# matschiner/navier-stokes-solver

Measured on AMD Instinct MI355X. Metric: Krylov iters/sec, 3D SIMPLE Stokes solve (BPCG), higher is better.
Workload: dtype f64

## Files before the change

### navier-stokes-solver_amd/csrc/bpcg2.hip

```cpp
#include "dist.h"


namespace nss {

enum { S_WD = 0, S_AS = 1, S_WDN = 2, S_ALPHA = 3, S_BETA = 4, S_ERR0 = 5, S_TOL = 6, S_REL = 7, S_WD_ODD = 8,
       S_AS_LOCAL = 9, S_WDN_LOCAL = 10 };
__device__ __forceinline__ int wd_slot(int it) { return (it & 1) ? S_WD_ODD : S_WD; }
enum { C_DONE = 0, C_IT_FINAL = 1, C_LAST_IT = 2, C_BREAKDOWN = 3, C_PENDING = 4, C_COMPUTED = 5, C_CLOSED = 6 };

struct EpiK1 {
  const int32_t* __restrict__ ctrl;
  const double* __restrict__ scal;
  double* __restrict__ u0;
  double* __restrict__ q;
  double* __restrict__ z0;
  const double* __restrict__ t2;
  double* __restrict__ s0;
  const double* __restrict__ w0;
  double* __restrict__ t0;
  double* __restrict__ t1;
  const double* __restrict__ dinv;
  double k;
  int it;
  __device__ bool skip() const { return ctrl[C_DONE] != 0; }
// ... 296 lines not shown
      u.x = fma(alpha, sv.x, u.x);
      u.y = fma(alpha, sv.y, u.y);
      double2 dn, wn;
      dn.x = fma(-alpha, t3v.x, d.x);
      dn.y = fma(-alpha, t3v.y, d.y);
      wn.x = fma(-alpha, mv.x * t3v.x, w.x);
      wn.y = fma(-alpha, mv.y * t3v.y, w.y);
      *reinterpret_cast<double2*>(a.u1 + i0) = u;
      *reinterpret_cast<double2*>(a.d1 + i0) = dn;
      *reinterpret_cast<double2*>(a.w1 + i0) = wn;
      acc = fma(wn.x, dn.x, acc);
      acc = fma(wn.y, dn.y, acc);
    } else {
      for (int i = i0; i < i0 + 2 && i < a.n_p; ++i) {
        const double sv = a.s1[i], t3v = a.t3[i];
        a.u1[i] = fma(alpha, sv, a.u1[i]);
        const double dn = fma(-alpha, t3v, a.d1[i]);
        const double wn = fma(-alpha, a.minv[i] * t3v, a.w1[i]);
        a.d1[i] = dn;
        a.w1[i] = wn;
        acc = fma(wn, dn, acc);
      }
    }
  } else {
    const int first = wg - a.gu - a.gp, stride = (int(gridDim.x) - a.gu - a.gp) * kBlock;
    for (int i = first * kBlock + int(threadIdx.x); i < a.ghost_n; i += stride)
      a.ghost_w0[i] = fma(-alpha, a.t1[a.ghost_map ? a.ghost_map[i] : a.n_u + i], a.ghost_w0[i]);
    for (int i = first * kBlock + int(threadIdx.x); i < a.ghost_p_n; i += stride)
      a.ghost_w1[i] = fma(-alpha, a.ghost_minv[i] * a.ghost_t3[i], a.ghost_w1[i]);
    return;
  }
  store_block_partial(acc, wg, a.partials, lds);
}

__global__ __launch_bounds__(kBlock) void bpcg2_k5_kernel(int32_t* __restrict__ ctrl, double* __restrict__ scal,
                                                           double* __restrict__ hist, int32_t it, int32_t n_p,
                                                           double* __restrict__ s1, const double* __restrict__ w1,
                                                           int32_t ghost_n, double* __restrict__ ghost_s0,
                                                           const double* __restrict__ ghost_w0, int32_t ghost_p_n,
                                                           double* __restrict__ ghost_s1,
                                                           const double* __restrict__ ghost_w1) {
  if (ctrl[C_DONE] != 0) return;
  const double wd = scal[wd_slot(it)], wdn = scal[S_WDN];
  const double beta = wdn / wd;
  if (blockIdx.x == 0 && threadIdx.x == 0) {
    scal[S_BETA] = beta;
    scal[wd_slot(it + 1)] = wdn;
    const double err = sqrt(fabs(wd));
    hist[it] = err;
    ctrl[C_LAST_IT] = it;
    ctrl[C_CLOSED] = it + 1;
    const double bound = scal[S_TOL] * (scal[S_REL] != 0.0 ? scal[S_ERR0] : 1.0);
    if (err < bound) {
      ctrl[C_IT_FINAL] = it;
      ctrl[C_DONE] = 1;
    }
  }
  const int stride = gridDim.x * kBlock;
  for (int i = blockIdx.x * kBlock + threadIdx.x; i < n_p; i += stride) s1[i] = fma(beta, s1[i], w1[i]);
  for (int i = blockIdx.x * kBlock + threadIdx.x; i < ghost_n; i += stride) ghost_s0[i] = fma(beta, ghost_s0[i], ghost_w0[i]);
  for (int i = blockIdx.x * kBlock + threadIdx.x; i < ghost_p_n; i += stride) ghost_s1[i] = fma(beta, ghost_s1[i], ghost_w1[i]);
}

__global__ __launch_bounds__(kBlock) void bpcg2_flush_kernel(const int32_t* __restrict__ ctrl,
                                                              const double* __restrict__ scal, int32_t n_u,
                                                              const double* __restrict__ s0, double* __restrict__ u0) {
  if (ctrl[C_PENDING] == 0) return;
  const double alpha = scal[S_ALPHA];
  const int stride = gridDim.x * kBlock;
  for (int i = blockIdx.x * kBlock + threadIdx.x; i < n_u; i += stride) u0[i] = fma(alpha, s0[i], u0[i]);
}

__global__ void bpcg2_flush_done_kernel(int32_t* __restrict__ ctrl) { ctrl[C_PENDING] = 0; }

struct CloseArgs {
  int32_t* ctrl;
  double* scal;
  double* hist;
  const double* partials_c;
  int32_t nc;
  int32_t fold;
};

template <bool FOLD>
__device__ __forceinline__ bool close_iteration(const CloseArgs& a, int it, double* lds, double* beta_out) {
  const int prev = it - 1;
  double wdn;
  if constexpr (FOLD) wdn = fixed_sum_1024(a.partials_c, a.nc, a.partials_c, 0, lds);
  else wdn = a.scal[S_WDN];
  const double wd = a.scal[wd_slot(prev)];
  const double beta = wdn / wd;
  const double err = sqrt(fabs(wd));
  const double bound = a.scal[S_TOL] * (a.scal[S_REL] != 0.0 ? a.scal[S_ERR0] : 1.0);
  const bool stop = err < bound;
  if (blockIdx.x == 0 && threadIdx.x == 0) {
    a.scal[S_BETA] = beta;
    a.scal[wd_slot(it)] = wdn;
    if (FOLD) a.scal[S_WDN] = wdn;
    a.hist[prev] = err;
    a.ctrl[C_LAST_IT] = prev;
    a.ctrl[C_CLOSED] = it;
    if (stop) {
      a.ctrl[C_IT_FINAL] = prev;
      a.ctrl[C_DONE] = 1;
    }
  }
  *beta_out = beta;
  return !stop;
}

__global__ __launch_bounds__(kBlock) void bpcg2_close_kernel(CloseArgs a) {
  __shared__ double lds[kRedDoubles];
  if (a.ctrl[C_DONE] != 0) return;
  const int computed = a.ctrl[C_COMPUTED];
  if (a.ctrl[C_CLOSED] >= computed) return;
  double beta;
  if (a.fold) close_iteration<true>(a, computed, lds, &beta);
  else close_iteration<false>(a, computed, lds, &beta);
}

template <bool FOLD, bool NT = false>
struct EpiK1c {
  CloseArgs cl;
  double* __restrict__ u0;
  double* __restrict__ q;
  double* __restrict__ z0;
  const double* __restrict__ t2;
  double* __restrict__ s0;
  const double* __restrict__ w0;
  double* __restrict__ t0;
  double* __restrict__ t1;
  const double* __restrict__ dinv;
  double k;
  int it;
  const double* __restrict__ s1;
  const double* __restrict__ w1;
  int32_t ghost_n = 0;
  double* __restrict__ ghost_s0 = nullptr;
  const double* __restrict__ ghost_w0 = nullptr;
  const int32_t* __restrict__ jb_first = nullptr;
  const int32_t* __restrict__ jb_order = nullptr;
  const int32_t* __restrict__ jb_run = nullptr;
  const double* __restrict__ jb_packed = nullptr;
  int32_t jb_count = 0, jb_bs = 0;
  double alpha = 0.0, beta = 0.0;
  bool pending = false;
  __device__ bool skip() const { return cl.ctrl[C_DONE] != 0; }
  __device__ bool prologue(double* lds) {
    if (it == 0) return true;
    alpha = cl.scal[S_ALPHA];
    pending = cl.ctrl[C_PENDING] == it;
    return close_iteration<FOLD>(cl, it, lds, &beta);
  }
  struct X {
    const double* __restrict__ s1;
    const double* __restrict__ w1;
    double beta;
    bool first;
    static constexpr bool kStageable = false;
    static constexpr bool kStageablePair = true;
    __device__ const double* ptr() const { return s1; }
    __device__ const double* ptr2() const { return w1; }
    __device__ double pair(double s, double w) const { return first ? s : fma(beta, s, w); }
    __device__ double operator()(int c) const { return first ? s1[c] : fma(beta, s1[c], w1[c]); }
  };
  __device__ X xop(const double*) const { return X{s1, w1, beta, it == 0}; }
#ifndef NSS_K1C_PREFETCH
#define NSS_K1C_PREFETCH 0
#endif

#if NSS_K1C_PREFETCH
  struct Pre { double q = 0.0, z0 = 0.0, t2 = 0.0, s0 = 0.0, w0 = 0.0, u0 = 0.0; };
  __device__ Pre fetch(int r) const {
    if (it == 0) return Pre{q[r], 0.0, 0.0, 0.0, 0.0, 0.0};
    return Pre{q[r], z0[r], t2[r], s0[r], w0[r], u0[r]};
  }
  __device__ void row(int r, double bts, const Pre& p) const {
#else
  struct PreLate { double q, z0, t2, s0, w0, u0; };
  __device__ void row(int r, double bts) const {
    const PreLate p{ld1s<NT>(q + r), it ? ld1s<NT>(z0 + r) : 0.0, it ? ld1s<NT>(t2 + r) : 0.0, it ? s0[r] : 0.0,
                    it ? ld1s<NT>(w0 + r) : 0.0, (it && pending) ? ld1s<NT>(u0 + r) : 0.0};
#endif
    double qv = p.q;
    if (it != 0) {
      const double zo = p.z0, t2v = p.t2, so = p.s0;
      if (pending) NSS_ST(u0[r], fma(alpha, so, p.u0));
      qv = fma(-alpha, t2v, fma(beta, qv, zo));
      NSS_ST(z0[r], fma(-alpha, t2v, zo));
      NSS_ST(q[r], qv);
      NSS_ST3(s0[r], fma(beta, so, p.w0));
    }
    const double t = qv + bts;
    NSS_ST3(t0[r], t);
    if (dinv) t1[r] = k * (dinv[r] * t);
    if (jb_first) {
      extern __shared__ double k1_t0[];
      k1_t0[r & (kBlockRows - 1)] = t;
    }
  }
  __device__ void finish(int b, double*) const {
    if (jb_first && b >= 0) {
      extern __shared__ double k1_t0[];
      __syncthreads();
      bjac_rows_from_lds(jb_first, jb_order, jb_run, jb_packed, jb_count, jb_bs, b, k1_t0,
                         [&](int i, double s) { t1[i] = k * s; });
    }
    if (it == 0 || ghost_n == 0) return;
    const int stride = gridDim.x * kBlock;
    for (int i = blockIdx.x * kBlock + threadIdx.x; i < ghost_n; i += stride) ghost_s0[i] = fma(beta, ghost_s0[i], ghost_w0[i]);
  }
};

struct EpiK2c {
  const int32_t* __restrict__ ctrl;
  const double* __restrict__ t0;
  const double* __restrict__ s0;
  double* __restrict__ t2;
  double* __restrict__ partials;
  double acc = 0.0;
  __device__ bool skip() const { return ctrl[C_DONE] != 0; }
  struct Pre { double s0 = 0.0, t0 = 0.0; };
  __device__ Pre fetch(int r) const { return Pre{s0[r], t0[r]}; }
  __device__ void row(int r, double at1, const Pre& p) {
    NSS_ST(t2[r], at1);
    acc = fma(p.s0, at1 - p.t0, acc);
  }
  __device__ void finish(int b, double* lds) { store_block_partial(acc, b, partials, lds); }
};

struct EpiK3c {
  const int32_t* __restrict__ ctrl;
  const double* __restrict__ scal;
  const double* __restrict__ t1;
  const double* __restrict__ s0;
  double* __restrict__ s1;
  const double* __restrict__ w1;
  double* __restrict__ t3;
  double* __restrict__ partials;
  int it;
  int n_own;
  double acc = 0.0;
  double beta = 0.0;
  __device__ bool skip() const { return ctrl[C_DONE] != 0; }
  __device__ bool prologue(double*) {
    if (it != 0) beta = scal[S_BETA];
    return true;
  }
  struct X {
    const double* __restrict__ t1;
    const double* __restrict__ s0;
    static constexpr bool kStageable = false;
    static constexpr bool kStageablePair = true;
    __device__ const double* ptr() const { return t1; }
    __device__ const double* ptr2() const { return s0; }
    __device__ double pair(double a, double b) const { return a - b; }
    __device__ double operator()(int c) const { return t1[c] - s0[c]; }
  };
  __device__ X xop(const double*) const { return X{t1, s0}; }
  struct Pre { double s1 = 0.0, w1 = 0.0; };
  __device__ Pre fetch(int r) const { return Pre{s1[r], it != 0 ? w1[r] : 0.0}; }
  __device__ void row(int r, double bt4, const Pre& p) {
    double sv = p.s1;
    if (it != 0) {
      sv = fma(beta, p.s1, p.w1);
      s1[r] = sv;
    }
    NSS_ST2(t3[r], bt4);
    if (r < n_own) acc = fma(sv, bt4, acc);
  }
  __device__ void finish(int b, double* lds) { store_block_partial(acc, b, partials, lds); }
};

static int k4_gu(const nss_bpcg2_t& s) { return (s.n_u + kK4PerBlock - 1) / kK4PerBlock; }
static int k4_gp(const nss_bpcg2_t& s) { return (s.n_p + kK4PerBlock - 1) / kK4PerBlock; }
static int k4_partials(const nss_bpcg2_t& s) { return k4_gu(s) + k4_gp(s); }
static int k4_ghost_blocks(const nss_bpcg2_t& s) {
  const int64_t g = std::max<int64_t>(s.ghost_mode ? s.ghost_n : 0, s.ghost_p_mode ? s.ghost_p_n : 0);
  return g > 0 ? stream_grid(g, kBlock) : 0;
}

constexpr int kFoldMax = 1024;
static int g_fold_mode = -1;
static bool fold_sums(const nss_bpcg2_t& s) {
  const int forced = g_fold_mode;
  if (s.local_sums) return false;
  if (forced >= 0) return forced != 0;
  return s.A->nblk + s.B->nblk <= kFoldMax && k4_partials(s) <= kFoldMax;
}

static void launch_k4(const nss_bpcg2_t& s, int it, bool fold, hipStream_t st) {
// ... 169 lines not shown
    launch_csr(*s.cond_HT, s.t0, EpiLift{s.ctrl, s.t0, s.cond_f}, st);
    src = s.cond_f;
  }
  const PreA p = pre_a_of(s);
  if (p.term() || p.bjac || s.cond_HT) pre_a_apply(p, s.k, src, s.t1, s.t2, s.ctrl, st);
  if (s.cond_HT) {
    if (cond_slab) cond_exchange(s, *d, d->cond_ext, 2, st);
    launch_csr(*s.cond_H, s.t1, EpiExtendInPlace{s.ctrl, s.t1}, st);
    launch_csr(*s.cond_inner, s.cond_f, EpiAddGuarded{s.ctrl, s.t1}, st);
  }
}

void bpcg2_phase(const nss_bpcg2_t& s, int which, int it, hipStream_t st) {
  switch (which) {
    case NSS_BPCG2_K1:
      bpcg2_spmv_phase(s, which, it, st, 0, -1);
      bpcg2_k1_finish(s, st);
      break;
    case NSS_BPCG2_K2:
    case NSS_BPCG2_K3:
      bpcg2_spmv_phase(s, which, it, st, 0, -1);
      break;
    case NSS_BPCG2_SUM1:
      if (s.p2p)
        hipLaunchKernelGGL(bpcg2_sum_p2p_kernel, dim3(1), dim3(kSumLanes), 0, st, s.ctrl, s.A->nblk, s.partials_a, s.B->nblk,
                           s.partials_b, s.scal, int(S_AS), int(S_AS_LOCAL), it, s.p2p->view(++s.p2p->seq));
      else
        hipLaunchKernelGGL(bpcg2_sum_kernel, dim3(1), dim3(kSumLanes), 0, st, s.ctrl, s.A->nblk, s.partials_a, s.B->nblk,
                           s.partials_b, s.scal, int(s.local_sums ? S_AS_LOCAL : S_AS));
      NSS_CHECK_LAUNCH();
      break;
    case NSS_BPCG2_ALPHA:
      break;
    case NSS_BPCG2_K4:
      if (s.dist_compact) throw Error("bpcg2: a state laid out for the compact partitioned plan takes the compact phases only");
      if (s.ghost_p_mode && s.ghost_p_n > 0)
        launch_csr(*s.ghost_b, s.t4, EpiGuardedStore{s.ctrl, s.ghost_t3}, st);
      launch_k4(s, it, false, st);
      break;
    case NSS_BPCG2_SUM2:
      if (s.p2p)
        hipLaunchKernelGGL(bpcg2_sum_p2p_kernel, dim3(1), dim3(kSumLanes), 0, st, s.ctrl, k4_partials(s), s.partials_c, 0,
                           s.partials_c, s.scal, int(S_WDN), int(S_WDN_LOCAL), it, s.p2p->view(++s.p2p->seq));
      else
        hipLaunchKernelGGL(bpcg2_sum_kernel, dim3(1), dim3(kSumLanes), 0, st, s.ctrl, k4_partials(s), s.partials_c, 0,
                           s.partials_c, s.scal, int(s.local_sums ? S_WDN_LOCAL : S_WDN));
      NSS_CHECK_LAUNCH();
      break;
    case NSS_BPCG2_BETA:
      break;
    case NSS_BPCG2_K5:
      if (s.dist_compact) throw Error("bpcg2: a state laid out for the compact partitioned plan takes the compact phases only");
      hipLaunchKernelGGL(bpcg2_k5_kernel, dim3(stream_grid(s.n_p, kBlock * 4)), dim3(kBlock), 0, st, s.ctrl, s.scal,
                         s.hist, it, s.n_p, s.s1, s.w1, s.ghost_mode ? s.ghost_n : 0, s.ghost_s0, s.ghost_w0,
                         s.ghost_p_mode ? s.ghost_p_n : 0, s.s1 + s.n_p, s.ghost_w1);
      NSS_CHECK_LAUNCH();
      break;
    default:
      throw Error("bpcg2: unknown phase");
  }
}

static CloseArgs close_args(const nss_bpcg2_t& s, bool fold) {
  return CloseArgs{s.ctrl, s.scal, s.hist, s.partials_c, k4_partials(s), fold ? 1 : 0};
}

constexpr int kFuseBjacMaxRows = 1 << 18;
static int g_fuse_bjac = -1;
bool fuse_block_jacobi_wanted(int64_t rows) { return g_fuse_bjac == 1 || (g_fuse_bjac == -1 && rows <= kFuseBjacMaxRows); }
bool c1_applies_block_jacobi(const nss_bpcg2_t& s) {
  return fuse_block_jacobi_wanted(s.n_u) && s.pre_bjac && !s.pre_bjac->gs_mat && !s.pre_amg && !s.pre_dist_amg && !s.pre_dist_aux && !s.pre_diag &&
         !s.cond_HT && s.BT->jb_first && s.BT->jb_serial == s.pre_bjac->serial && s.pre_bjac->inv_sym && s.pre_bjac->run;
}

void bpcg2_cphase(const nss_bpcg2_t& s, int which, int it, hipStream_t st, const nss_dist_s* d) {
  const bool fold = fold_sums(s);
  switch (which) {
    case NSS_BPCG2C_C1: {
      const double* dinv = (s.pre_amg || s.pre_dist_amg || s.pre_dist_aux || s.cond_HT) ? nullptr : s.pre_diag;
      const bool nt = s.BT->ell_col != nullptr && stream_vector_loads(s.n_u);
      const bool fj = c1_applies_block_jacobi(s);
      const nss_bjac_s* J = s.pre_bjac;
      const size_t lds = fj ? sizeof(double) * kBlockRows : 0;
#define NSS_C1(FOLD, NT, LAUNCH)                                                                                       \
  LAUNCH<kCodes>(*s.BT, s.s1, EpiK1c<FOLD, NT>{close_args(s, FOLD), s.u0, s.q, s.z0, s.t2, s.s0, s.w0, s.t0, s.t1, dinv, s.k, it, \
                                       s.s1, s.w1, s.dist_compact ? s.ghost_n : 0, s.ghost_s0, s.ghost_w0,                 \
                                       fj ? s.BT->jb_first : nullptr, fj ? s.BT->jb_order : nullptr, fj ? J->run : nullptr, fj ? J->inv_sym : nullptr,   \
                                       fj ? J->nblocks : 0, fj ? J->bs : 0}, st, 0, -1, lds)
      if (nt && fold) NSS_C1(true, true, launch_csr_direct);
      else if (nt) NSS_C1(false, true, launch_csr_direct);
      else if (fold) NSS_C1(true, false, launch_csr);
      else NSS_C1(false, false, launch_csr);
#undef NSS_C1
      if (!fj) bpcg2_k1_finish(s, st, d);
      break;
    }
    case NSS_BPCG2C_C23: {
      EpiK2c ea{s.ctrl, s.t0, s.s0, s.t2, s.partials_a};
      EpiK3c eb{s.ctrl, s.scal, s.t1, s.s0, s.s1, s.w1, s.t3, s.partials_b, it, s.n_p};
      if (!launch_csr_dual<kCodes>(*s.A, s.t1, ea, *s.B, s.t1, eb, st)) {
        launch_csr<kCodes>(*s.A, s.t1, ea, st);
        launch_csr<kCodes>(*s.B, s.t1, eb, st);
      }
      break;
    }
    case NSS_BPCG2C_SUMA:
      if (!fold) bpcg2_phase(s, NSS_BPCG2_SUM1, it, st);
      break;
    case NSS_BPCG2C_C4:
      launch_k4(s, it, fold, st);
      break;
    case NSS_BPCG2C_SUMW:
      if (!fold) bpcg2_phase(s, NSS_BPCG2_SUM2, it, st);
      break;
    default:
      throw Error("bpcg2: unknown phase of the compact plan");
  }
}

}

using namespace nss;

extern "C" {

int nss_bpcg2_workspace(const nss_bpcg2_t* s, int64_t* partials_a, int64_t* partials_b, int64_t* partials_c) {
  return guarded([&] {
    NSS_REQUIRE(s && s->A && s->B, "bpcg2_workspace: NULL state / matrices");
    int64_t need[3];
    bpcg2_need(*s, need);
    if (partials_a) *partials_a = need[0];
    if (partials_b) *partials_b = need[1];
    if (partials_c) *partials_c = need[2];
  });
}

int nss_bpcg2_phase(const nss_bpcg2_t* s, int32_t which, int32_t it, nss_stream_t stream) {
  return guarded([&] {
    bpcg2_check_state(s);
    bpcg2_phase(*s, which, it, as_stream(stream));
  });
}

int nss_bpcg2_phases(const nss_bpcg2_t* s, int32_t first, int32_t last, int32_t it, nss_stream_t stream) {
  return guarded([&] {
    bpcg2_check_state(s);
    NSS_REQUIRE(first >= NSS_BPCG2_K1 && last <= NSS_BPCG2_K5 && first <= last, "bpcg2_phases: bad phase range");
    for (int ph = first; ph <= last; ++ph) bpcg2_phase(*s, ph, it, as_stream(stream));
  });
}

int nss_bpcg2_iterate(const nss_bpcg2_t* s, int32_t it_begin, int32_t it_end, nss_stream_t stream) {
  return guarded([&] {
    bpcg2_check_state(s);
    hipStream_t st = as_stream(stream);
    NSS_REQUIRE(!s->ghost_mode && !s->ghost_p_mode && !s->local_sums,
                "bpcg2_iterate: a row-partitioned state takes nss_bpcg2_phase / nss_bpcg2_iterate_dist");
    for (int it = it_begin; it < it_end; ++it)
      for (int ph = NSS_BPCG2C_C1; ph <= NSS_BPCG2C_SUMW; ++ph) bpcg2_cphase(*s, ph, it, st);
  });
}

int nss_bpcg2_iterate_classic(const nss_bpcg2_t* s, int32_t it_begin, int32_t it_end, nss_stream_t stream) {
  return guarded([&] {
    bpcg2_check_state(s);
    hipStream_t st = as_stream(stream);
    for (int it = it_begin; it < it_end; ++it)
      for (int ph = NSS_BPCG2_K1; ph <= NSS_BPCG2_K5; ++ph) bpcg2_phase(*s, ph, it, st);
  });
}

int nss_bpcg2_cphases(const nss_bpcg2_t* s, int32_t first, int32_t last, int32_t it, nss_stream_t stream) {
  return guarded([&] {
    bpcg2_check_state(s);
    NSS_REQUIRE(first >= NSS_BPCG2C_C1 && last <= NSS_BPCG2C_SUMW && first <= last, "bpcg2_cphases: bad phase range");
// ... 63 lines not shown
```

### navier-stokes-solver_amd/csrc/csr_stream.h

```cpp
#pragma once

#include <type_traits>
#include <vector>

#include "nss_common.h"

#include <initializer_list>
#include <string>

namespace nss {

#ifndef NSS_STREAM_NT
#define NSS_STREAM_NT 1
#endif

#ifndef NSS_STREAM_PREFETCH
#define NSS_STREAM_PREFETCH 1
#endif

#ifndef NSS_PREFETCH_ROWS
#define NSS_PREFETCH_ROWS 1
#endif

#ifndef NSS_CHUNK
// ... 403 lines not shown
          if (RG > 1) {
#pragma unroll
            for (int off = RG / 2; off > 0; off >>= 1) sum += __shfl_xor(sum, off, kWave);
          }
          if (sub == 0) EpiPre<Epi>::row(epi, r, sum, pf.pre[q]);
        }
      }
      for (int r = rf + kPF * kRowsPerPass; r < r1; r += kRowsPerPass) {
        const int s = a.rowptr[r] - p0;
        const int e = a.rowptr[r + 1] - p0;
        double sum = 0.0;
        for (int j = s + sub; j < e; j += RG) sum += prod[j];
        if (RG > 1) {
#pragma unroll
          for (int off = RG / 2; off > 0; off >>= 1) sum += __shfl_xor(sum, off, kWave);
        }
        if (sub == 0) EpiPre<Epi>::row(epi, r, sum, EpiPre<Epi>::fetch(epi, r));
      }
#else
      for (int r = r0 + tid / RG; r < r1; r += kRowsPerPass) {
        const int s = a.rowptr[r] - p0;
        const int e = a.rowptr[r + 1] - p0;
        double sum = 0.0;
        for (int j = s + sub; j < e; j += RG) sum += prod[j];
        if (RG > 1) {
#pragma unroll
          for (int off = RG / 2; off > 0; off >>= 1) sum += __shfl_xor(sum, off, kWave);
        }
        if (sub == 0) EpiPre<Epi>::row(epi, r, sum, EpiPre<Epi>::fetch(epi, r));
      }
#endif
    } else {
      if (!EpiPrologue<Epi>::run(epi, red)) return;
      const XOp xop = EpiX<Epi>::get(epi, x);
      double acc = 0.0;
      const typename StoredValue<VT>::type* __restrict__ vals = view_values<VT>(a);
      if constexpr (std::is_same<VT, Coded8>::value) {
        asm volatile("s_waitcnt vmcnt(0)" ::: "memory");
        __syncthreads();
      }
      for (int i = tid; i < cnt; i += kBlock) acc = fma(value_of<VT>(vals[p0 + i], dict), xop(a.col[p0 + i]), acc);
      const double sum = block_sum(acc, red);
      if (tid == 0) EpiPre<Epi>::row(epi, r0, sum, EpiPre<Epi>::fetch(epi, r0));
    }
  }
  epi.finish(b, red);
}

template <int RG, class Epi, int IDX = 0, int CH = kChunk, bool GRP = false, class VT = double>
__global__ __launch_bounds__(kBlock) void csr_stream_kernel(CsrView a, const double* __restrict__ x, Epi epi) {
  __shared__ double prod[CH];
  __shared__ double red[kRedDoubles];
  __shared__ int32_t window[kWindows];
  if (epi.skip()) return;
  csr_stream_body<RG, Epi, IDX, CH, GRP, VT>(a, x, epi, int(blockIdx.x), prod, red, window);
}

#ifndef NSS_DUAL_SECOND_FIRST
#define NSS_DUAL_SECOND_FIRST 1
#endif
template <int RG, class EpiA, class EpiB, int IDXA, int IDXB, int CH, bool GRP, class VT = double>
__global__ __launch_bounds__(kBlock) void csr_stream_dual_kernel(CsrView a, CsrView b, int grid_a, int grid_b,
                                                                  const double* __restrict__ xa,
                                                                  const double* __restrict__ xb, EpiA ea, EpiB eb) {
  __shared__ double prod[CH];
  __shared__ double red[kRedDoubles];
  __shared__ int32_t window[kWindows];
#if NSS_DUAL_SECOND_FIRST
  const bool first = int(blockIdx.x) >= grid_b;
  const int wg = first ? int(blockIdx.x) - grid_b : int(blockIdx.x);
#else
  const bool first = int(blockIdx.x) < grid_a;
  const int wg = first ? int(blockIdx.x) : int(blockIdx.x) - grid_a;
#endif
  if (first) {
    if (ea.skip()) return;
    csr_stream_body<RG, EpiA, IDXA, CH, (GRP && IDXA != 0), VT>(a, xa, ea, wg, prod, red, window);
  } else {
    if (eb.skip()) return;
    csr_stream_body<RG, EpiB, IDXB, CH, (GRP && IDXB != 0), VT>(b, xb, eb, wg, prod, red, window);
  }
}

template <class Epi, class VT = double>
__global__ __launch_bounds__(kBlock) void csr_direct_kernel(CsrView a, const int32_t* __restrict__ ecol,
                                                            const double* __restrict__ eval,
                                                            const uint16_t* __restrict__ ecode,
                                                            const double* __restrict__ x, Epi epi) {
  static_assert(kDirectWidth == 2, "csr_direct_kernel is written for two slots per row");
  using XOp = typename EpiX<Epi>::type;
  constexpr bool kCoded = std::is_same<VT, Coded8>::value;
  __shared__ double red[kRedDoubles];
  double* const dict = DictLds<VT>::get();
  if (epi.skip()) return;
  const int tid = threadIdx.x, wg = int(blockIdx.x);
  const int lb = (wg & (kXcds - 1)) * a.per_xcd + (wg >> 3);
  const int b = lb < a.nblk ? a.blk0 + lb : -1;
  if (b >= 0) {
    DictLds<VT>::request(a, dict);
    const int r0 = a.rowblk[b], r1 = a.rowblk[b + 1];
    for (int base = r0; base < r1; base += kDirectRows) {
      constexpr int kRows = kDirectRows / kBlock;
      typedef int32_t int2v __attribute__((ext_vector_type(2)));
      int2v c[kRows];
      dbl2v v[kRows];
      uint16_t code[kRows];
      typename EpiPre<Epi>::type pre[kRows];
#pragma unroll
      for (int q = 0; q < kRows; ++q) {
        const int r = base + tid + q * kBlock;
        const bool live = r < r1;
        c[q] = live ? __builtin_nontemporal_load(reinterpret_cast<const int2v*>(ecol) + r) : int2v{-1, -1};
        if constexpr (kCoded) code[q] = live ? __builtin_nontemporal_load(ecode + r) : uint16_t(0);
        else v[q] = live ? __builtin_nontemporal_load(reinterpret_cast<const dbl2v*>(eval) + r) : dbl2v{0.0, 0.0};
        pre[q] = live ? EpiPre<Epi>::fetch(epi, r) : typename EpiPre<Epi>::type{};
      }
      if (base == r0 && !EpiPrologue<Epi>::run(epi, red)) return;
      const XOp xop = EpiX<Epi>::get(epi, x);
      double x0[kRows], x1[kRows];
#pragma unroll
      for (int q = 0; q < kRows; ++q) {
        x0[q] = c[q].x >= 0 ? xop(c[q].x) : 0.0;
        x1[q] = c[q].y >= 0 ? xop(c[q].y) : 0.0;
      }
      if constexpr (kCoded) {
        asm volatile("s_waitcnt vmcnt(0)" ::: "memory");
        __syncthreads();
#pragma unroll
        for (int q = 0; q < kRows; ++q) v[q] = dbl2v{dict[code[q] & 0xff], dict[code[q] >> 8]};
      }
#pragma unroll
      for (int q = 0; q < kRows; ++q) {
        const int r = base + tid + q * kBlock;
        if (r < r1) {
          double sum = 0.0;
          if (c[q].x >= 0) sum += mul_unfused(v[q].x, x0[q]);
          if (c[q].y >= 0) sum += mul_unfused(v[q].y, x1[q]);
          EpiPre<Epi>::row(epi, r, sum, pre[q]);
        }
      }
    }
  }
  epi.finish(b, red);
}

enum : unsigned { kF64 = 0, kF32 = 1, kCodes = 2 };

template <int I>
using Idx = std::integral_constant<int, I>;
template <class VT>
struct ValueTag { using type = VT; };
template <class VT>
constexpr bool kHasGroupedForms = !std::is_same<VT, Coded8>::value;

template <class F>
inline void for_plan_lanes(const nss_csr_s& A, F&& f) {
  switch (A.rg) {
    case 1: f(Idx<1>{}); break;
    case 2: f(Idx<2>{}); break;
    case 4: f(Idx<4>{}); break;
    case 8: f(Idx<8>{}); break;
    case 16: f(Idx<16>{}); break;
    case 32: f(Idx<32>{}); break;
    case 64: f(Idx<64>{}); break;
    default: throw Error("csr_stream: bad lanes-per-row in the launch plan");
  }
}

template <class VT, class Epi>
inline void launch_csr_stream_kernel(const nss_csr_s& A, const double* x, const Epi& epi, hipStream_t st, int b0, int b1,
                                     size_t dyn_lds) {
  constexpr bool kCanStage = EpiX<Epi>::type::kStageable;
  constexpr bool kCanPair = XPairable<typename EpiX<Epi>::type>::value;
  const int mode = A.idx_mode(kCanStage, kCanPair);
  const bool grp = mode != 0 && A.gb > 1;
  const CsrView v = A.view(b0, b1, mode, std::is_same<VT, float>::value);
  const dim3 grid(nss_csr_s::grid(b1 - b0)), block(kBlock);
  for_plan_lanes(A, [&](auto lanes) {
    const auto go = [&](auto idx) {
      constexpr int RG = decltype(lanes)::value, IDX = decltype(idx)::value;
      constexpr bool kGrp = IDX != 0 && kHasGroupedForms<VT>;
      if (kGrp && grp) hipLaunchKernelGGL((csr_stream_kernel<RG, Epi, IDX, kChunk, kGrp, VT>), grid, block, dyn_lds, st, v, x, epi);
      else hipLaunchKernelGGL((csr_stream_kernel<RG, Epi, IDX, kChunk, false, VT>), grid, block, dyn_lds, st, v, x, epi);
    };
    if (mode == 2) { if constexpr (kCanStage) go(Idx<2>{}); }
    else if (mode == 3) { if constexpr (kCanPair) go(Idx<3>{}); }
    else if (mode == 1) go(Idx<1>{});
    else go(Idx<0>{});
  });
  NSS_CHECK_LAUNCH();
}

template <unsigned FORMS = kF64, bool DIRECT_ONLY = false, class Epi>
inline void launch_csr(const nss_csr_s& A, const double* x, const Epi& epi, hipStream_t st, int b0 = 0, int b1 = -1,
                       size_t dyn_lds = 0) {
  constexpr bool kF32Form = (FORMS & kF32) != 0 && !DIRECT_ONLY, kCodedForm = (FORMS & kCodes) != 0;
  using CodedVT = std::conditional_t<kCodedForm, Coded8, double>;
  if (b1 < 0) b1 = A.nblk;
  if (A.m == 0 || b1 <= b0) return;
  if constexpr (kF32Form) {
    if (A.val32) {
      NSS_REQUIRE(!A.ell_col, "csr_stream: a matrix with fp32 values has no fixed-width copy");
      launch_csr_stream_kernel<float>(A, x, epi, st, b0, b1, dyn_lds);
      return;
    }
  }
  if (DIRECT_ONLY && !A.ell_col) throw Error("csr_direct: the matrix has no fixed-width copy");
  if (A.ell_col) {
    const dim3 grid(nss_csr_s::grid(b1 - b0)), block(kBlock);
    const CsrView v = A.view(b0, b1, 0);
    if (kCodedForm && A.coded() && A.ell_code)
      hipLaunchKernelGGL((csr_direct_kernel<Epi, CodedVT>), grid, block, dyn_lds, st, v, A.ell_col, A.ell_val, A.ell_code, x, epi);
    else
      hipLaunchKernelGGL((csr_direct_kernel<Epi>), grid, block, dyn_lds, st, v, A.ell_col, A.ell_val, (const uint16_t*)nullptr, x, epi);
    NSS_CHECK_LAUNCH();
  } else if constexpr (!DIRECT_ONLY) {
    if (kCodedForm && A.coded() && !A.val32) launch_csr_stream_kernel<CodedVT>(A, x, epi, st, b0, b1, dyn_lds);
    else launch_csr_stream_kernel<double>(A, x, epi, st, b0, b1, dyn_lds);
  }
}

template <unsigned FORMS = kF64, class Epi>
inline void launch_csr_direct(const nss_csr_s& A, const double* x, const Epi& epi, hipStream_t st, int b0 = 0,
                              int b1 = -1, size_t dyn_lds = 0) {
// ... 88 lines not shown
```

### navier-stokes-solver_amd/csrc/spmv.hip

```cpp
#include "bpcg2.h"
#include "code_keys.h"
#include "csr_stream.h"
#include "precond.h"

#include <algorithm>
#include <climits>
#include <vector>

namespace nss {

#ifndef NSS_PLAN_FILL_CHIP
#define NSS_PLAN_FILL_CHIP 1
#endif
constexpr int kMinRowBlocks = 2048;

#ifndef NSS_DIRECT_MIN_ROWS
#define NSS_DIRECT_MIN_ROWS (1 << 21)
#endif

static int64_t g_direct_min_rows = NSS_DIRECT_MIN_ROWS;

static int g_pair_mode = -1;
bool pair_staging_enabled() { return g_pair_mode != 0; }

// ... 621 lines not shown
  (void)hipFree(A.ell_code);
  A.val8 = nullptr;
  A.dict = nullptr;
  A.ell_code = nullptr;
  A.dict_count = 0;
}

bool collect_patterns(int64_t n, const double* val, std::vector<unsigned long long>& keys, hipStream_t st) {
  keys.clear();
  if (n <= 0) return false;
  unsigned long long* table = nullptr;
  int32_t* state = nullptr;
  int32_t h_state[4] = {0, 1, 0, 0};
  std::vector<unsigned long long> h_table(kCodeSlots);
  try {
    NSS_HIP(hipMalloc(&table, sizeof(unsigned long long) * kCodeSlots));
    NSS_HIP(hipMalloc(&state, sizeof(int32_t) * 4));
    NSS_HIP(hipMemsetAsync(table, 0xff, sizeof(unsigned long long) * kCodeSlots, st));
    NSS_HIP(hipMemsetAsync(state, 0, sizeof(int32_t) * 4, st));
    hipLaunchKernelGGL(code_collect_kernel, dim3(stream_grid(n, kBlock * 8)), dim3(kBlock), 0, st, n, val, table, state);
    NSS_CHECK_LAUNCH();
    NSS_HIP(hipMemcpyAsync(h_state, state, sizeof h_state, hipMemcpyDeviceToHost, st));
    NSS_HIP(hipMemcpyAsync(h_table.data(), table, sizeof(unsigned long long) * kCodeSlots, hipMemcpyDeviceToHost, st));
    NSS_HIP(hipStreamSynchronize(st));
  } catch (...) {
    (void)hipFree(table);
    (void)hipFree(state);
    throw;
  }
  (void)hipFree(table);
  (void)hipFree(state);
  return code_keys_from_table(h_table.data(), kCodeSlots, h_state, size_t(kDictSize), keys);
}

void assign_pattern_codes(int64_t n, const double* val, const std::vector<unsigned long long>& keys, uint8_t* codes,
                          hipStream_t st) {
  unsigned long long* d_keys = nullptr;
  try {
    NSS_HIP(hipMalloc(&d_keys, sizeof(unsigned long long) * kDictSize));
    NSS_HIP(hipMemcpyAsync(d_keys, keys.data(), sizeof(unsigned long long) * keys.size(), hipMemcpyHostToDevice, st));
    hipLaunchKernelGGL(code_assign_kernel, dim3(stream_grid(n, kBlock * 8)), dim3(kBlock), 0, st, n, val, d_keys,
                       int(keys.size()), codes);
    NSS_CHECK_LAUNCH();
    NSS_HIP(hipStreamSynchronize(st));
  } catch (...) {
    (void)hipFree(d_keys);
    throw;
  }
  (void)hipFree(d_keys);
}

static bool code_values(nss_csr_s& A, hipStream_t st) {
  if (A.val8) return true;
  if (A.val32 || !A.val || A.nnz == 0) return false;
  if (A.gb > 1) return false;
  std::vector<unsigned long long> keys;
  if (!collect_patterns(A.nnz, A.val, keys, st)) return false;
  uint8_t* val8 = nullptr;
  double* dict = nullptr;
  try {
    std::vector<unsigned long long> h_dict(kDictSize, 0ull);
    std::copy(keys.begin(), keys.end(), h_dict.begin());
    NSS_HIP(hipMalloc(&dict, sizeof(double) * kDictSize));
    NSS_HIP(hipMalloc(&val8, size_t(A.nnz) + 4));
    NSS_HIP(hipMemsetAsync(val8, 0, size_t(A.nnz) + 4, st));
    NSS_HIP(hipMemcpyAsync(dict, h_dict.data(), sizeof(double) * kDictSize, hipMemcpyHostToDevice, st));
    assign_pattern_codes(A.nnz, A.val, keys, val8, st);
  } catch (...) {
    (void)hipFree(val8);
    (void)hipFree(dict);
    throw;
  }
  A.val8 = val8;
  A.dict = dict;
  A.dict_count = int32_t(keys.size());
  build_ell_code(A, st);
  return true;
}

static void direct_rows(nss_csr_s& A, hipStream_t st) {
#if NSS_DIRECT_ROWS
  if (A.val32) return;
  if (A.m < g_direct_min_rows || A.nnz > int64_t(kDirectWidth) * A.m) return;
  int32_t* ecol = nullptr;
  double* eval = nullptr;
  int32_t* wide = nullptr;
  try {
    NSS_HIP(hipMalloc(&ecol, sizeof(int32_t) * size_t(A.m) * kDirectWidth));
    NSS_HIP(hipMalloc(&eval, sizeof(double) * size_t(A.m) * kDirectWidth));
    NSS_HIP(hipMalloc(&wide, sizeof(int32_t)));
    NSS_HIP(hipMemsetAsync(wide, 0, sizeof(int32_t), st));
    hipLaunchKernelGGL(ell_build_kernel, dim3(stream_grid(A.m, kBlock * 4)), dim3(kBlock), 0, st, A.m, A.rowptr, A.col,
                       A.val, ecol, eval, wide);
    NSS_CHECK_LAUNCH();
    int32_t h_wide = 1;
    NSS_HIP(hipMemcpyAsync(&h_wide, wide, sizeof(int32_t), hipMemcpyDeviceToHost, st));
    NSS_HIP(hipStreamSynchronize(st));
    if (h_wide == 0) {
      A.ell_col = ecol;
      A.ell_val = eval;
      ecol = nullptr;
      eval = nullptr;
      build_ell_code(A, st);
    }
  } catch (...) {
    (void)hipFree(ecol);
    (void)hipFree(eval);
    (void)hipFree(wide);
    throw;
  }
  (void)hipFree(ecol);
  (void)hipFree(eval);
  (void)hipFree(wide);
#else
  (void)A;
  (void)st;
#endif
}

void compress_columns(nss_csr_s& A, hipStream_t st) {
#if NSS_COL16
  if (A.nnz == 0 || A.nblk == 0) return;
  stage_columns(A, st);
  window_columns(A, st);
  group_columns(A, st);
  direct_rows(A, st);
  if (!A.ell_col) build_dispatch(A, st);
#else
  (void)A;
  (void)st;
#endif
}

__global__ __launch_bounds__(kBlock) void round_f32_kernel(int64_t n, const double* __restrict__ in, double* out64,
                                                            float* __restrict__ out32) {
  const int64_t stride = int64_t(gridDim.x) * kBlock;
  for (int64_t i = int64_t(blockIdx.x) * kBlock + threadIdx.x; i < n; i += stride) {
    const float v = float(in[i]);
    if (out32) out32[i] = v;
    else out64[i] = double(v);
  }
}

__global__ __launch_bounds__(kBlock) void csr_diag_kernel(int32_t m, const int32_t* __restrict__ rowptr,
                                                           const int32_t* __restrict__ col,
                                                           const double* __restrict__ val, double* __restrict__ d) {
  const int r = blockIdx.x * kBlock + threadIdx.x;
  if (r >= m) return;
  double v = 0.0;
  for (int p = rowptr[r]; p < rowptr[r + 1]; ++p)
    if (col[p] == r) v = val[p];
  d[r] = v;
}

}

using namespace nss;

extern "C" {

int nss_csr_create(int32_t nrows, int32_t ncols, int64_t nnz, const int32_t* h_rowptr, const int32_t* h_col,
                   const double* h_val, nss_csr_t* out) {
  return nss_csr_create_cuts(nrows, ncols, nnz, h_rowptr, h_col, h_val, 0, nullptr, out);
}

int nss_csr_create_cuts(int32_t nrows, int32_t ncols, int64_t nnz, const int32_t* h_rowptr, const int32_t* h_col,
// ... 446 lines not shown
```

Measured before the change: 2427.

## Specialize C1 direct kernel on first iteration and use scalar uniform loads

Adds a compile-time IT0 template parameter to the K1 epilogue so the first-iteration and steady-state paths are instantiated separately, and routes the C1 phase through the direct ELL kernel whenever ell_col exists. Control and scalar reads are issued through constant address space so they can become scalar loads. The direct kernel is split into a helper with a full-block fast path that clamps row indices instead of predicating loads, and it always prefetches the epilogue operands. The trade-offs are more template instances, extra loads for rows past the end and unconditional u0 reads, plus a guard against empty-column matrices.

```diff
diff --git a/navier-stokes-solver_amd/csrc/bpcg2.hip b/navier-stokes-solver_amd/csrc/bpcg2.hip
--- a/navier-stokes-solver_amd/csrc/bpcg2.hip
+++ b/navier-stokes-solver_amd/csrc/bpcg2.hip
@@ -402,16 +402,24 @@
   int32_t fold;
 };
 
+__device__ __forceinline__ int32_t uniform_i32(const int32_t* p, int i) {
+  return ((const int32_t __attribute__((address_space(4)))*)p)[i];
+}
+__device__ __forceinline__ double uniform_f64(const double* p, int i) {
+  return ((const double __attribute__((address_space(4)))*)p)[i];
+}
+
 template <bool FOLD>
 __device__ __forceinline__ bool close_iteration(const CloseArgs& a, int it, double* lds, double* beta_out) {
   const int prev = it - 1;
   double wdn;
   if constexpr (FOLD) wdn = fixed_sum_1024(a.partials_c, a.nc, a.partials_c, 0, lds);
-  else wdn = a.scal[S_WDN];
-  const double wd = a.scal[wd_slot(prev)];
+  else wdn = uniform_f64(a.scal, S_WDN);
+  const double wd = uniform_f64(a.scal, wd_slot(prev));
   const double beta = wdn / wd;
   const double err = sqrt(fabs(wd));
-  const double bound = a.scal[S_TOL] * (a.scal[S_REL] != 0.0 ? a.scal[S_ERR0] : 1.0);
+  const double rel = uniform_f64(a.scal, S_REL), err0 = uniform_f64(a.scal, S_ERR0);
+  const double bound = uniform_f64(a.scal, S_TOL) * (rel != 0.0 ? err0 : 1.0);
   const bool stop = err < bound;
   if (blockIdx.x == 0 && threadIdx.x == 0) {
     a.scal[S_BETA] = beta;
@@ -439,7 +447,7 @@
   else close_iteration<false>(a, computed, lds, &beta);
 }
 
-template <bool FOLD, bool NT = false>
+template <bool FOLD, bool NT = false, int IT0 = -1>
 struct EpiK1c {
   CloseArgs cl;
   double* __restrict__ u0;
@@ -465,11 +473,12 @@
   int32_t jb_count = 0, jb_bs = 0;
   double alpha = 0.0, beta = 0.0;
   bool pending = false;
-  __device__ bool skip() const { return cl.ctrl[C_DONE] != 0; }
+  __device__ bool first() const { return IT0 < 0 ? it == 0 : IT0 == 1; }
+  __device__ bool skip() const { return uniform_i32(cl.ctrl, C_DONE) != 0; }
   __device__ bool prologue(double* lds) {
-    if (it == 0) return true;
-    alpha = cl.scal[S_ALPHA];
-    pending = cl.ctrl[C_PENDING] == it;
+    if (first()) return true;
+    alpha = uniform_f64(cl.scal, S_ALPHA);
+    pending = uniform_i32(cl.ctrl, C_PENDING) == it;
     return close_iteration<FOLD>(cl, it, lds, &beta);
   }
   struct X {
@@ -482,28 +491,27 @@
     __device__ const double* ptr() const { return s1; }
     __device__ const double* ptr2() const { return w1; }
     __device__ double pair(double s, double w) const { return first ? s : fma(beta, s, w); }
-    __device__ double operator()(int c) const { return first ? s1[c] : fma(beta, s1[c], w1[c]); }
+    __device__ double operator()(int c) const {
+      if constexpr (IT0 == 1) return s1[c];
+      else if constexpr (IT0 == 0) return fma(beta, s1[c], w1[c]);
+      else return first ? s1[c] : fma(beta, s1[c], w1[c]);
+    }
   };
-  __device__ X xop(const double*) const { return X{s1, w1, beta, it == 0}; }
-#ifndef NSS_K1C_PREFETCH
-#define NSS_K1C_PREFETCH 0
-#endif
-
-#if NSS_K1C_PREFETCH
-  struct Pre { double q = 0.0, z0 = 0.0, t2 = 0.0, s0 = 0.0, w0 = 0.0, u0 = 0.0; };
-  __device__ Pre fetch(int r) const {
-    if (it == 0) return Pre{q[r], 0.0, 0.0, 0.0, 0.0, 0.0};
-    return Pre{q[r], z0[r], t2[r], s0[r], w0[r], u0[r]};
-  }
-  __device__ void row(int r, double bts, const Pre& p) const {
-#else
-  struct PreLate { double q, z0, t2, s0, w0, u0; };
+  __device__ X xop(const double*) const { return X{s1, w1, beta, first()}; }
+  struct Ops { double q, z0, t2, s0, w0, u0; };
+  using DirectPre = Ops;
+  __device__ Ops fetch_direct(int r) const {
+    if constexpr (IT0 == 1) return Ops{ld1s<NT>(q + r), 0.0, 0.0, 0.0, 0.0, 0.0};
+    else return Ops{ld1s<NT>(q + r), ld1s<NT>(z0 + r), ld1s<NT>(t2 + r), s0[r], ld1s<NT>(w0 + r), ld1s<NT>(u0 + r)};
+  }
   __device__ void row(int r, double bts) const {
-    const PreLate p{ld1s<NT>(q + r), it ? ld1s<NT>(z0 + r) : 0.0, it ? ld1s<NT>(t2 + r) : 0.0, it ? s0[r] : 0.0,
-                    it ? ld1s<NT>(w0 + r) : 0.0, (it && pending) ? ld1s<NT>(u0 + r) : 0.0};
-#endif
+    const bool it = !first();
+    row(r, bts, Ops{ld1s<NT>(q + r), it ? ld1s<NT>(z0 + r) : 0.0, it ? ld1s<NT>(t2 + r) : 0.0, it ? s0[r] : 0.0,
+                    it ? ld1s<NT>(w0 + r) : 0.0, (it && pending) ? ld1s<NT>(u0 + r) : 0.0});
+  }
+  __device__ void row(int r, double bts, const Ops& p) const {
     double qv = p.q;
-    if (it != 0) {
+    if (!first()) {
       const double zo = p.z0, t2v = p.t2, so = p.s0;
       if (pending) NSS_ST(u0[r], fma(alpha, so, p.u0));
       qv = fma(-alpha, t2v, fma(beta, qv, zo));
@@ -526,7 +534,7 @@
       bjac_rows_from_lds(jb_first, jb_order, jb_run, jb_packed, jb_count, jb_bs, b, k1_t0,
                          [&](int i, double s) { t1[i] = k * s; });
     }
-    if (it == 0 || ghost_n == 0) return;
+    if (first() || ghost_n == 0) return;
     const int stride = gridDim.x * kBlock;
     for (int i = blockIdx.x * kBlock + threadIdx.x; i < ghost_n; i += stride) ghost_s0[i] = fma(beta, ghost_s0[i], ghost_w0[i]);
   }
@@ -862,15 +870,25 @@
       const bool fj = c1_applies_block_jacobi(s);
       const nss_bjac_s* J = s.pre_bjac;
       const size_t lds = fj ? sizeof(double) * kBlockRows : 0;
-#define NSS_C1(FOLD, NT, LAUNCH)                                                                                       \
-  LAUNCH<kCodes>(*s.BT, s.s1, EpiK1c<FOLD, NT>{close_args(s, FOLD), s.u0, s.q, s.z0, s.t2, s.s0, s.w0, s.t0, s.t1, dinv, s.k, it, \
+#define NSS_C1(FOLD, NT, IT0, LAUNCH)                                                                                  \
+  LAUNCH<kCodes>(*s.BT, s.s1, EpiK1c<FOLD, NT, IT0>{close_args(s, FOLD), s.u0, s.q, s.z0, s.t2, s.s0, s.w0, s.t0, s.t1, dinv, s.k, it, \
                                        s.s1, s.w1, s.dist_compact ? s.ghost_n : 0, s.ghost_s0, s.ghost_w0,                 \
                                        fj ? s.BT->jb_first : nullptr, fj ? s.BT->jb_order : nullptr, fj ? J->run : nullptr, fj ? J->inv_sym : nullptr,   \
                                        fj ? J->nblocks : 0, fj ? J->bs : 0}, st, 0, -1, lds)
-      if (nt && fold) NSS_C1(true, true, launch_csr_direct);
-      else if (nt) NSS_C1(false, true, launch_csr_direct);
-      else if (fold) NSS_C1(true, false, launch_csr);
-      else NSS_C1(false, false, launch_csr);
+      if (s.BT->ell_col) {
+        const int sel = (fold ? 4 : 0) + (nt ? 2 : 0) + (it == 0 ? 1 : 0);
+        switch (sel) {
+          case 0: NSS_C1(false, false, 0, launch_csr_direct); break;
+          case 1: NSS_C1(false, false, 1, launch_csr_direct); break;
+          case 2: NSS_C1(false, true, 0, launch_csr_direct); break;
+          case 3: NSS_C1(false, true, 1, launch_csr_direct); break;
+          case 4: NSS_C1(true, false, 0, launch_csr_direct); break;
+          case 5: NSS_C1(true, false, 1, launch_csr_direct); break;
+          case 6: NSS_C1(true, true, 0, launch_csr_direct); break;
+          default: NSS_C1(true, true, 1, launch_csr_direct); break;
+        }
+      } else if (fold) NSS_C1(true, false, -1, launch_csr);
+      else NSS_C1(false, false, -1, launch_csr);
 #undef NSS_C1
       if (!fj) bpcg2_k1_finish(s, st, d);
       break;
diff --git a/navier-stokes-solver_amd/csrc/csr_stream.h b/navier-stokes-solver_amd/csrc/csr_stream.h
--- a/navier-stokes-solver_amd/csrc/csr_stream.h
+++ b/navier-stokes-solver_amd/csrc/csr_stream.h
@@ -509,64 +509,98 @@
   }
 }
 
+template <class E, class = void>
+struct EpiDirectPre : EpiPre<E> {};
+template <class E>
+struct EpiDirectPre<E, std::void_t<typename E::DirectPre>> {
+  using type = typename E::DirectPre;
+  static __device__ type fetch(const E& e, int r) { return e.fetch_direct(r); }
+  static __device__ void row(E& e, int r, double ax, const type& p) { e.row(r, ax, p); }
+};
+
+template <bool FULL, class Epi, class VT>
+__device__ __forceinline__ bool csr_direct_rows(const CsrView& a, const int32_t* __restrict__ ecol,
+                                                const double* __restrict__ eval, const uint16_t* __restrict__ ecode,
+                                                const double* __restrict__ x, Epi& epi, int base, int r1, bool base_first,
+                                                double* red, double* dict) {
+  using XOp = typename EpiX<Epi>::type;
+  using Pre = EpiDirectPre<Epi>;
+  constexpr bool kCoded = std::is_same<VT, Coded8>::value;
+  constexpr int kRows = kDirectRows / kBlock;
+  typedef int32_t int2v __attribute__((ext_vector_type(2)));
+  const int tid = threadIdx.x;
+  int rl[kRows];
+#pragma unroll
+  for (int q = 0; q < kRows; ++q) {
+    const int r = base + tid + q * kBlock;
+    rl[q] = FULL ? r : (r < r1 ? r : r1 - 1);
+  }
+  int2v c[kRows];
+  dbl2v v[kRows];
+  uint16_t code[kRows];
+  typename Pre::type pre[kRows];
+#pragma unroll
+  for (int q = 0; q < kRows; ++q) c[q] = __builtin_nontemporal_load(reinterpret_cast<const int2v*>(ecol) + rl[q]);
+#pragma unroll
+  for (int q = 0; q < kRows; ++q) {
+    if constexpr (kCoded) code[q] = __builtin_nontemporal_load(ecode + rl[q]);
+    else v[q] = __builtin_nontemporal_load(reinterpret_cast<const dbl2v*>(eval) + rl[q]);
+  }
+#pragma unroll
+  for (int q = 0; q < kRows; ++q) pre[q] = Pre::fetch(epi, rl[q]);
+  if (base_first) DictLds<VT>::request(a, dict);
+  if (base_first && !EpiPrologue<Epi>::run(epi, red)) return false;
+  const XOp xop = EpiX<Epi>::get(epi, x);
+  double x0[kRows], x1[kRows];
+#pragma unroll
+  for (int q = 0; q < kRows; ++q) {
+    x0[q] = xop(c[q].x >= 0 ? c[q].x : 0);
+    x1[q] = xop(c[q].y >= 0 ? c[q].y : 0);
+  }
+  if constexpr (kCoded) {
+    asm volatile("s_waitcnt vmcnt(0)" ::: "memory");
+    __syncthreads();
+#pragma unroll
+    for (int q = 0; q < kRows; ++q) v[q] = dbl2v{dict[code[q] & 0xff], dict[code[q] >> 8]};
+  }
+#pragma unroll
+  for (int q = 0; q < kRows; ++q) {
+    const int r = base + tid + q * kBlock;
+    const double p0 = mul_unfused(v[q].x, x0[q]), p1 = mul_unfused(v[q].y, x1[q]);
+    double sum = 0.0;
+    sum += c[q].x >= 0 ? p0 : 0.0;
+    sum += c[q].y >= 0 ? p1 : 0.0;
+    if (FULL || r < r1) Pre::row(epi, r, sum, pre[q]);
+  }
+  return true;
+}
+
 template <class Epi, class VT = double>
 __global__ __launch_bounds__(kBlock) void csr_direct_kernel(CsrView a, const int32_t* __restrict__ ecol,
                                                             const double* __restrict__ eval,
                                                             const uint16_t* __restrict__ ecode,
                                                             const double* __restrict__ x, Epi epi) {
   static_assert(kDirectWidth == 2, "csr_direct_kernel is written for two slots per row");
-  using XOp = typename EpiX<Epi>::type;
-  constexpr bool kCoded = std::is_same<VT, Coded8>::value;
   __shared__ double red[kRedDoubles];
   double* const dict = DictLds<VT>::get();
   if (epi.skip()) return;
-  const int tid = threadIdx.x, wg = int(blockIdx.x);
+  const int wg = int(blockIdx.x);
   const int lb = (wg & (kXcds - 1)) * a.per_xcd + (wg >> 3);
   const int b = lb < a.nblk ? a.blk0 + lb : -1;
   if (b >= 0) {
-    DictLds<VT>::request(a, dict);
-    const int r0 = a.rowblk[b], r1 = a.rowblk[b + 1];
-    for (int base = r0; base < r1; base += kDirectRows) {
-      constexpr int kRows = kDirectRows / kBlock;
-      typedef int32_t int2v __attribute__((ext_vector_type(2)));
-      int2v c[kRows];
-      dbl2v v[kRows];
-      uint16_t code[kRows];
-      typename EpiPre<Epi>::type pre[kRows];
-#pragma unroll
-      for (int q = 0; q < kRows; ++q) {
-        const int r = base + tid + q * kBlock;
-        const bool live = r < r1;
-        c[q] = live ? __builtin_nontemporal_load(reinterpret_cast<const int2v*>(ecol) + r) : int2v{-1, -1};
-        if constexpr (kCoded) code[q] = live ? __builtin_nontemporal_load(ecode + r) : uint16_t(0);
-        else v[q] = live ? __builtin_nontemporal_load(reinterpret_cast<const dbl2v*>(eval) + r) : dbl2v{0.0, 0.0};
-        pre[q] = live ? EpiPre<Epi>::fetch(epi, r) : typename EpiPre<Epi>::type{};
-      }
-      if (base == r0 && !EpiPrologue<Epi>::run(epi, red)) return;
-      const XOp xop = EpiX<Epi>::get(epi, x);
-      double x0[kRows], x1[kRows];
-#pragma unroll
-      for (int q = 0; q < kRows; ++q) {
-        x0[q] = c[q].x >= 0 ? xop(c[q].x) : 0.0;
-        x1[q] = c[q].y >= 0 ? xop(c[q].y) : 0.0;
-      }
-      if constexpr (kCoded) {
-        asm volatile("s_waitcnt vmcnt(0)" ::: "memory");
-        __syncthreads();
-#pragma unroll
-        for (int q = 0; q < kRows; ++q) v[q] = dbl2v{dict[code[q] & 0xff], dict[code[q] >> 8]};
-      }
-#pragma unroll
-      for (int q = 0; q < kRows; ++q) {
-        const int r = base + tid + q * kBlock;
-        if (r < r1) {
-          double sum = 0.0;
-          if (c[q].x >= 0) sum += mul_unfused(v[q].x, x0[q]);
-          if (c[q].y >= 0) sum += mul_unfused(v[q].y, x1[q]);
-          EpiPre<Epi>::row(epi, r, sum, pre[q]);
-        }
-      }
-    }
+    typedef const int32_t __attribute__((address_space(4))) * ConstI32;
+    const ConstI32 rb = (ConstI32)(a.rowblk + b);
+    const int r0 = rb[0], r1 = rb[1];
+    bool go = true;
+    if (r1 - r0 == kDirectRows) {
+      go = csr_direct_rows<true, Epi, VT>(a, ecol, eval, ecode, x, epi, r0, r1, true, red, dict);
+    } else if (r1 - r0 < kDirectRows) {
+      if (r1 > r0) go = csr_direct_rows<false, Epi, VT>(a, ecol, eval, ecode, x, epi, r0, r1, true, red, dict);
+    } else {
+      for (int base = r0; go && base < r1; base += kDirectRows)
+        go = csr_direct_rows<false, Epi, VT>(a, ecol, eval, ecode, x, epi, base, r1, base == r0, red, dict);
+    }
+    if (!go) return;
   }
   epi.finish(b, red);
 }
diff --git a/navier-stokes-solver_amd/csrc/spmv.hip b/navier-stokes-solver_amd/csrc/spmv.hip
--- a/navier-stokes-solver_amd/csrc/spmv.hip
+++ b/navier-stokes-solver_amd/csrc/spmv.hip
@@ -727,6 +727,7 @@
 #if NSS_DIRECT_ROWS
   if (A.val32) return;
   if (A.m < g_direct_min_rows || A.nnz > int64_t(kDirectWidth) * A.m) return;
+  if (A.n == 0) return;
   int32_t* ecol = nullptr;
   double* eval = nullptr;
   int32_t* wide = nullptr;
```

Result: faster. 2560, median of 6 (+5.5%).
